# ethz-asl/okvis

Hardware: AMD Instinct MI355X
Metric: Gauss-Newton iterations/sec on 10-KF x 2-cam x 400-landmark windows (batch throughput: window-iterations/s) (higher is better)
Workload: dtype f64

## Files before the change

okvis_amd/csrc/ba_linearize2.hpp:

```cpp
#pragma once
#include "ba_linearize.hpp"

namespace ba {

constexpr int LIN2_REC = 27;
constexpr int LIN2_POSES = 64;
constexpr int LIN2_CAMS = 8;
constexpr int LIN2_IDX_INTS = 2 * (((GROUP_LM + 1) + 2 * LIN2_PIECES + LIN_TASK_CACHE * 6 + LIN2_PIECES / 2 + LIN2_PIECES / 4 + LIN2_CAMS + 1) / 2);

template <class REAL, bool FUSE, int UB = LIN2_REC>
struct Lin2Cfg {
  static constexpr int PAIR_REC_DOUBLES = (LIN2_PIECES * (UB > 16 ? UB : 16) * (int)sizeof(REAL) + 7) / 8;
  static constexpr int STAGE = LinCfg<false, REAL>::STAGE_DOUBLES;
  static constexpr int REC_DOUBLES = FUSE ? (STAGE > PAIR_REC_DOUBLES ? STAGE : PAIR_REC_DOUBLES) : PAIR_REC_DOUBLES;
  static constexpr int FIXED_DOUBLES = REC_DOUBLES + GROUP_LM * 4 + GROUP_LM * 16 + 4 * 64 + LIN2_POSES * 7 + LIN2_CAMS * 12 + LIN2_IDX_INTS / 2;
  static constexpr int MIN_STEP_DOUBLES = FUSE ? 1024 : 0;
};
static_assert(LIN2_PIECES * 3 * 2 <= LIN2_PIECES * 16, "phase A's pair sums alias the record area");
static_assert(LIN2_PIECES <= LIN_THREADS, "one pair per work-item");
__device__ __forceinline__ float fma_real(float a, float b, float c) { return fmaf(a, b, c); }
__device__ __forceinline__ double fma_real(double a, double b, double c) { return fma(a, b, c); }
template <class T>
__device__ __forceinline__ T sub_of_rounded_products(T a, T b, T c, T d) {
#pragma clang fp contract(off)
  const T p = a * b, q = c * d;
  return p - q;
}

template <class T>
__device__ __forceinline__ T row_next(T v) { return quad_xchg<0x101>(v); }
__device__ __forceinline__ int row_next_i(int v, int old) { return __builtin_amdgcn_update_dpp(old, v, 0x101, 0xF, 0xF, false); }
__device__ __forceinline__ int row_prev_i(int v, int old) { return __builtin_amdgcn_update_dpp(old, v, 0x111, 0xF, 0xF, false); }

struct Lin2Ops {
  ObsRec rec;
  int lpb, pp, poff, plm, pblock, slot;
  Task task;
};
struct Lin2Heavy {
  double Wp0[18];
  double bb[3], v[6], xx[4], sl[3];
  int lp0, lp1;
};

template <class REAL, bool FUSE, bool SMALL, int OCC = 2, int UB = LIN2_REC>
__global__ __launch_bounds__(LIN_THREADS, OCC) void linearize2_kernel(const WinPtrs* __restrict__ wins, const OptD* __restrict__ optp, int init,
                                                                      int n_small, int step_doubles) {
  extern __shared__ __attribute__((aligned(16))) double smem[];
  const WinPtrs& W = wins[blockIdx.y];
  int wg = blockIdx.x;
  if constexpr (SMALL) {
    if ((int)blockIdx.x < n_small) {
      small_body(W, init, blockIdx.x, smem);
      return;
    }
    wg -= n_small;
  }
  const int g = wg;
  if (g >= W.n_group) return;
#define LSTAMP(k) do { if (W.prof && threadIdx.x == 0 && g == 0) W.prof[k] = (double)clock64(); } while (0)
  const Ctrl* ctrl = W.ctrl;
  if (ctrl->done) return;
  const OptD opt = *optp;
  constexpr int RECD = Lin2Cfg<REAL, FUSE, UB>::REC_DOUBLES;
  REAL* s_rec = reinterpret_cast<REAL*>(smem);
  double* s_pair = smem;
  double* s_lm = smem + RECD;
  double* s_lmres = s_lm + GROUP_LM * 4;
  double* s_sc = s_lmres + GROUP_LM * 16;
  double* s_pose = s_sc + 4 * 64;
  double* s_cam = s_pose + LIN2_POSES * 7;
  int* s_lpb = reinterpret_cast<int*>(s_cam + LIN2_CAMS * 12);
  int* s_pp = s_lpb + GROUP_LM + 1;
  int* s_poff = s_pp + LIN2_PIECES;
  int* s_task = s_poff + LIN2_PIECES;
  int* s_cmodel = s_task + LIN_TASK_CACHE * 6;
  uint16_t* s_slot = reinterpret_cast<uint16_t*>(s_cmodel + LIN2_CAMS);
  uint8_t* s_plm = reinterpret_cast<uint8_t*>(s_slot + LIN2_PIECES);
  double* s_step = reinterpret_cast<double*>(s_lpb + LIN2_IDX_INTS);
  double* s_aux = s_step + (step_doubles - Lin2Cfg<REAL, FUSE, UB>::MIN_STEP_DOUBLES);
  const int tid = threadIdx.x, lane = tid & 63, wave = tid >> 6;

  auto reduce_own_group = [&](int g, int buf, double lam) {
    const Group Gr = W.groups[g];
    const int trows = min(TILE_DIM, W.Dp);
    double* tables = smem;
    double* aux = s_aux;
    double(*vinv)[6] = reinterpret_cast<double(*)[6]>(aux);
    double(*bvec)[3] = reinterpret_cast<double(*)[3]>(aux + SCHUR_CHUNK_LM_MAX * 6);
    int* boff = reinterpret_cast<int*>(aux + SCHUR_CHUNK_LM_MAX * 9);
    const SchurPairBeginGlobal pb{W.lm_pair_begin, Gr.lm_begin, Gr.lm_end};
    const int n_tp = W.n_tile * (W.n_tile + 1) / 2;
    for (int tp = 0; tp < n_tp; ++tp) {
      schur_reduce_chunk(W, opt, g, tp, Gr.lm_begin, Gr.lm_end, buf, lam, trows, tables, vinv, bvec, boff, pb, g == 0 && blockIdx.y == 0);
      __syncthreads();
    }
  };
  if (!init && !ctrl->pending) {
    if constexpr (FUSE)
      reduce_own_group(g, ctrl->acc, opt.dogleg ? ctrl->mu : 1.0 / ctrl->radius);
    return;
  }
  const int acc = ctrl->acc, trial = 1 - acc;
  const double lambda = ctrl->lambda;
  const double lam_next = opt.dogleg ? ((init || ctrl->first || opt.gauss_newton) ? ctrl->mu : fmax(DL_MIN_MU, 2.0 * ctrl->mu / DL_MU_INCREASE))
                                     : 1.0 / ctrl->radius;
  const bool dl_explicit = opt.dogleg && ctrl->tr_kind == 1;
  const double dl_cA = ctrl->cA, dl_beta = ctrl->beta;
  const bool fast = FUSE && W.fuse_fast;
  const bool poses_staged = W.n_pose <= LIN2_POSES, cams_staged = W.n_cam <= LIN2_CAMS;

  {
    const double* ps = W.pose[trial];
    const int np7 = 7 * min(W.n_pose, LIN2_POSES);
    for (int i = tid; i < np7; i += LIN_THREADS) s_pose[i] = ps[i];
    const int nc = min(W.n_cam, LIN2_CAMS);
    if (tid < 12 * nc) s_cam[tid] = W.cam_intr[tid];
    if (tid < nc) s_cmodel[tid] = W.cam_model[tid];
  }

  auto issue_loads = [&](const Group& G, Lin2Ops& o) {
    const int nlm = G.lm_end - G.lm_begin, nobs = G.obs_end - G.obs_begin, npair = G.pair_end - G.pair_begin, ntask = G.task_end - G.task_begin;
    o.rec.lm_cam = 0; o.rec.pose = 0; o.rec.ext = 0; o.rec.u = 0; o.rec.v = 0; o.rec.sw = 0;
    if (tid < nobs) o.rec = W.obs[G.obs_begin + tid];
    o.lpb = o.pp = o.poff = o.plm = o.pblock = o.slot = 0;
    if (tid <= nlm) o.lpb = W.lm_piece_begin[G.lm_begin + tid] - G.piece_begin;
    if (tid < npair) {
      o.pp = W.pair_piece[G.pair_begin + tid];
      o.poff = W.pair_off[G.pair_begin + tid];
      o.plm = W.pair_lm[G.pair_begin + tid] - G.lm_begin;
      o.pblock = W.pair_block[G.pair_begin + tid];
      o.slot = W.task_list[G.tlist_begin + tid];
    }
    if (ntask <= LIN_TASK_CACHE && tid < ntask) o.task = W.tasks[G.task_begin + tid];
  };
  auto issue_heavy = [&](const Group& G, Lin2Heavy& o) {
    const int nlm = G.lm_end - G.lm_begin, npair = G.pair_end - G.pair_begin;
    o.sl[0] = o.sl[1] = o.sl[2] = 1.0;
    o.lp0 = o.lp1 = 0;
    if (!init) {
      if (tid < npair) {
        const double* Wp = W.W[acc] + (size_t)(G.pair_begin + tid) * 18;
#pragma unroll
        for (int i = 0; i < 18; ++i) o.Wp0[i] = Wp[i];
      }
      if (tid < nlm) {
        const int l = G.lm_begin + tid;
        const double* b = W.bl[acc] + 3 * (size_t)l;
        const double* Vl = W.V[acc] + 6 * (size_t)l;
        const double* x = W.lm[acc] + 4 * (size_t)l;
#pragma unroll
        for (int i = 0; i < 3; ++i) o.bb[i] = b[i];
#pragma unroll
        for (int i = 0; i < 6; ++i) o.v[i] = Vl[i];
#pragma unroll
        for (int i = 0; i < 4; ++i) o.xx[i] = x[i];
        o.lp0 = W.lm_pair_begin[l] - G.pair_begin;
        o.lp1 = W.lm_pair_begin[l + 1] - G.pair_begin;
        if (opt.dogleg) {
          const double* sl = W.lm_scale + 3 * (size_t)l;
          o.sl[0] = sl[0], o.sl[1] = sl[1], o.sl[2] = sl[2];
        }
      }
    } else if (tid < nlm) {
      const double* x = W.lm[trial] + 4 * (size_t)(G.lm_begin + tid);
#pragma unroll
      for (int i = 0; i < 4; ++i) o.xx[i] = x[i];
    }
  };

  const Group G = W.groups[g];
  Lin2Ops ops;
  issue_loads(G, ops);
  if (!init)
    for (int i = tid; i < W.Dp; i += LIN_THREADS) s_step[i] = W.step[i];

  {
    LSTAMP(40);
    Lin2Heavy hv;
    issue_heavy(G, hv);
    const int nlm = G.lm_end - G.lm_begin;
    const int nobs = G.obs_end - G.obs_begin;
    const int npair = G.pair_end - G.pair_begin;
    const int ntask = G.task_end - G.task_begin;
    const bool has_obs = tid < nobs, has_pair = tid < npair;
    const bool tasks_cached = ntask <= LIN_TASK_CACHE;
    const ObsRec rec = ops.rec;
    const int pf_poff = ops.poff, pf_plm = ops.plm, pf_pblock = ops.pblock;
    double pf_sc[3] = {1.0, 1.0, 1.0};
    if (fast && !init && tid >= 64 && tid - 64 < nlm) {
      const double* sl = W.lm_scale + 3 * (size_t)(G.lm_begin + tid - 64);
      pf_sc[0] = sl[0], pf_sc[1] = sl[1], pf_sc[2] = sl[2];
    }
    LSTAMP(41);
    if (!init) {
      __syncthreads();
      if (has_pair) {
        const double* d = s_step + pf_poff;
        double t0 = 0, t1 = 0, t2 = 0;
#pragma unroll
        for (int i = 0; i < 6; ++i) {
          t0 += hv.Wp0[3 * i] * d[i];
          t1 += hv.Wp0[3 * i + 1] * d[i];
          t2 += hv.Wp0[3 * i + 2] * d[i];
        }
        s_pair[3 * tid] = t0;
        s_pair[3 * tid + 1] = t1;
        s_pair[3 * tid + 2] = t2;
      }
      __syncthreads();
      double sc_gd = 0, sc_ddd = 0, sc_s2 = 0, sc_x2 = 0;
      if (tid < nlm) {
        const int l = G.lm_begin + tid;
        double t[3] = {hv.bb[0], hv.bb[1], hv.bb[2]};
        for (int p = hv.lp0; p < hv.lp1; ++p) {
          const double* sp = s_pair + 3 * p;
          t[0] += sp[0];
          t[1] += sp[1];
          t[2] += sp[2];
        }
        double v[6] = {hv.v[0], hv.v[1], hv.v[2], hv.v[3], hv.v[4], hv.v[5]};
        const double d0 = damp_diag(v[0], hv.sl[0], opt);
        const double d1 = damp_diag(v[3], hv.sl[1], opt);
        const double d2 = damp_diag(v[5], hv.sl[2], opt);
        v[0] += lambda * d0;
        v[3] += lambda * d1;
        v[5] += lambda * d2;
        double vi[6];
        inv3sym(v, vi);
        const double dl0 = -(vi[0] * t[0] + vi[1] * t[1] + vi[2] * t[2]);
        const double dl1 = -(vi[1] * t[0] + vi[3] * t[1] + vi[4] * t[2]);
        const double dl2 = -(vi[2] * t[0] + vi[4] * t[1] + vi[5] * t[2]);
        double st0 = dl0, st1 = dl1, st2 = dl2;
        if (dl_explicit) {
          st0 = -dl_cA * (hv.bb[0] / d0) + dl_beta * dl0;
          st1 = -dl_cA * (hv.bb[1] / d1) + dl_beta * dl1;
          st2 = -dl_cA * (hv.bb[2] / d2) + dl_beta * dl2;
        }
        const double x0 = hv.xx[0], x1 = hv.xx[1], x2 = hv.xx[2], x3 = hv.xx[3];
        double* xt = W.lm[trial] + 4 * (size_t)l;
        const double n0 = x0 + st0, n1 = x1 + st1, n2 = x2 + st2;
        xt[0] = n0; xt[1] = n1; xt[2] = n2; xt[3] = x3;
        s_lm[4 * tid] = n0; s_lm[4 * tid + 1] = n1; s_lm[4 * tid + 2] = n2; s_lm[4 * tid + 3] = x3;
        sc_gd = hv.bb[0] * dl0 + hv.bb[1] * dl1 + hv.bb[2] * dl2;
        sc_ddd = d0 * dl0 * dl0 + d1 * dl1 * dl1 + d2 * dl2 * dl2;
        sc_s2 = st0 * st0 + st1 * st1 + st2 * st2;
        sc_x2 = x0 * x0 + x1 * x1 + x2 * x2 + x3 * x3;
      }
      if (tid < 64) {
        s_sc[tid] = sc_gd;
        s_sc[64 + tid] = sc_ddd;
        s_sc[128 + tid] = sc_s2;
        s_sc[192 + tid] = sc_x2;
      }
    } else {
      if (tid < nlm) {
        s_lm[4 * tid] = hv.xx[0]; s_lm[4 * tid + 1] = hv.xx[1]; s_lm[4 * tid + 2] = hv.xx[2]; s_lm[4 * tid + 3] = hv.xx[3];
      }
      if (tid < 64) s_sc[tid] = s_sc[64 + tid] = s_sc[128 + tid] = s_sc[192 + tid] = 0.0;
    }
    if (tid <= nlm) s_lpb[tid] = ops.lpb;
    if (has_pair) {
      s_pp[tid] = ops.pp;
      s_poff[tid] = pf_poff;
      s_plm[tid] = (uint8_t)pf_plm;
      s_slot[tid] = (uint16_t)ops.slot;
    }
    if (tasks_cached && tid < ntask) {
      int* t = s_task + 6 * tid;
      t[0] = ops.task.type; t[1] = ops.task.off_a; t[2] = ops.task.off_b;
      t[3] = ops.task.list_begin - G.tlist_begin; t[4] = ops.task.list_end - G.tlist_begin; t[5] = ops.task.out;
    }
    if (fast) {
      int* blktask = reinterpret_cast<int*>(s_aux + GROUP_LM * 9 + FUSE_MAX_TASKS * 36);
      if (tid >= 64 && tid < 64 + 32) blktask[tid - 64] = -1;
    }
    __syncthreads();
    LSTAMP(42);
    if (fast && tid < ntask) reinterpret_cast<int*>(s_aux + GROUP_LM * 9 + FUSE_MAX_TASKS * 36)[ops.task.off_a / 6] = tid;

    REAL a[16];
#pragma unroll
    for (int e = 0; e < 16; ++e) a[e] = REAL(0);
    const int key_l = has_obs ? (int)(rec.lm_cam & 0xFFFFFFu) : -1;
    const int key_p = has_obs ? (int)rec.pose : -1;
    if (has_obs) {
      const int o = G.obs_begin + tid;
      const int cam = (int)(rec.lm_cam >> 24);
      double P[7], E[7], intr[12];
      int cam_model;
      if (poses_staged) {
#pragma unroll
        for (int i = 0; i < 7; ++i) {
          P[i] = s_pose[7 * (int)rec.pose + i];
          E[i] = s_pose[7 * (int)rec.ext + i];
        }
      } else {
        const double* pose = W.pose[trial] + 7 * (size_t)rec.pose;
        const double* ext = W.pose[trial] + 7 * (size_t)rec.ext;
#pragma unroll
        for (int i = 0; i < 7; ++i) {
          P[i] = pose[i];
          E[i] = ext[i];
        }
      }
      if (cams_staged) {
#pragma unroll
        for (int i = 0; i < 12; ++i) intr[i] = s_cam[12 * cam + i];
        cam_model = s_cmodel[cam];
      } else {
#pragma unroll
        for (int i = 0; i < 12; ++i) intr[i] = W.cam_intr[12 * cam + i];
        cam_model = W.cam_model[cam];
      }
      const double* lm = s_lm + 4 * (key_l - G.lm_begin);
      const double L4[4] = {lm[0], lm[1], lm[2], lm[3]};
      REAL r0, r1, jl[6];
      if constexpr (std::is_same<REAL, double>::value) {
        ReprojLin Jd;
        reproj_linearize(P, E, L4, intr, cam_model, rec.u, rec.v, rec.sw, false, &Jd);
        r0 = Jd.r[0], r1 = Jd.r[1];
#pragma unroll
        for (int i = 0; i < 6; ++i) jl[i] = Jd.Jl[i];
      } else {
        ReprojLinT<REAL> J;
        reproj_linearize_mixed<REAL>(P, E, L4, intr, cam_model, rec.u, rec.v, rec.sw, false, &J);
        r0 = J.r[0], r1 = J.r[1];
#pragma unroll
        for (int i = 0; i < 6; ++i) jl[i] = J.Jl[i];
      }
      if (W.obs_r[trial]) {
        W.obs_r[trial][2 * (size_t)o] = r0;
        W.obs_r[trial][2 * (size_t)o + 1] = r1;
      }
      const REAL s = r0 * r0 + r1 * r1;
      REAL sr = REAL(1), irho = REAL(1), cost = REAL(0.5) * s;
      if (W.cauchy_b > 0) {
        const REAL bb = REAL(W.cauchy_b * W.cauchy_b);
        const REAL sum = REAL(1) + s / bb;
        const REAL rho1 = REAL(1) / sum;
        cost = REAL(0.5) * bb * log(sum);
        sr = sqrt(rho1);
        irho = sum;
      }
      r0 *= sr, r1 *= sr;
#pragma unroll
      for (int i = 0; i < 6; ++i) jl[i] *= sr;
      a[0] = jl[0] * jl[0] + jl[3] * jl[3];
      a[1] = jl[0] * jl[1] + jl[3] * jl[4];
      a[2] = jl[0] * jl[2] + jl[3] * jl[5];
      a[3] = jl[1] * jl[1] + jl[4] * jl[4];
      a[4] = jl[1] * jl[2] + jl[4] * jl[5];
      a[5] = jl[2] * jl[2] + jl[5] * jl[5];
      a[6] = jl[0] * r0 + jl[3] * r1;
      a[7] = jl[1] * r0 + jl[4] * r1;
      a[8] = jl[2] * r0 + jl[5] * r1;
#pragma unroll
      for (int e = 0; e < 6; ++e) a[9 + e] = a[e] * irho;
      a[15] = cost;
    }
    LSTAMP(43);
    const int prev_l = row_prev_i(key_l, -2), prev_p = row_prev_i(key_p, -2);
    const int next_l = row_next_i(key_l, -2), next_p = row_next_i(key_p, -2);
    const bool brk = ((lane & 15) == 0) | (key_l != prev_l) | (key_p != prev_p);
    const bool same_next = has_obs & ((lane & 15) != 15) & (key_l == next_l) & (key_p == next_p);
    const unsigned long long brk_mask = __ballot(brk);
    const unsigned long long below = brk_mask & ((2ull << lane) - 1ull);
    const int run_start = 63 - __builtin_clzll(below);
    const bool head = has_obs && (((lane - run_start) & 1) == 0);
    const bool merge = head && same_next;
    const unsigned long long head_mask = __ballot(head);
    const int pw = wave == 0 ? 0 : (wave == 1 ? G.pw1 : (wave == 2 ? G.pw2 : G.pw3));
    const int piece = pw + __builtin_amdgcn_mbcnt_hi((unsigned)(head_mask >> 32), __builtin_amdgcn_mbcnt_lo((unsigned)head_mask, 0));
#pragma unroll
    for (int e = 0; e < 16; ++e) {
      const REAL t = row_next(a[e]);
      a[e] += merge ? t : REAL(0);
    }
    if (head) {
      REAL* rp = s_rec + 16 * piece;
#pragma unroll
      for (int e = 0; e < 16; ++e) rp[e] = a[e];
    }
    __syncthreads();
    LSTAMP(44);

    {
      const int e = tid & 15;
      const bool is_cost = e == 15, is_b = e >= 6 && e < 9;
      double* obase = e < 6 ? W.V[trial] : (is_b ? W.bl[trial] : W.Hq[trial]);
      const int ostride = is_b ? 3 : 6, ooff = e < 6 ? e : (is_b ? e - 6 : e - 9);
      for (int wi = tid; wi < nlm * 16; wi += LIN_THREADS) {
        const int ll = wi >> 4;
        const int p0 = s_lpb[ll], p1 = s_lpb[ll + 1];
        REAL s0 = 0, s1 = 0;
        int p = p0;
        for (; p + 1 < p1; p += 2) {
          s0 += s_rec[16 * p + e];
          s1 += s_rec[16 * (p + 1) + e];
        }
        if (p < p1) s0 += s_rec[16 * p + e];
        const REAL sum = s0 + s1;
        if (!is_cost) obase[ostride * (size_t)(G.lm_begin + ll) + ooff] = sum;
        s_lmres[16 * ll + e] = sum;
        if (init && opt.dogleg && (e == 0 || e == 3 || e == 5))
          W.lm_scale[3 * (size_t)(G.lm_begin + ll) + (e == 0 ? 0 : (e == 3 ? 1 : 2))] = opt.jacobi_scaling ? 1.0 / (1.0 + sqrt((double)sum)) : 1.0;
      }
    }
    LSTAMP(45);
    REAL vp[6] = {0, 0, 0, 0, 0, 0}, bp[3] = {0, 0, 0};
    REAL d0 = 0, d1 = 0, d2 = 0, hw = 0;
    int my_slot = 0;
    if (has_pair) {
      const int pp = s_pp[tid];
      const int p0 = pp & 0xFFFF, p1 = p0 + (pp >> 16);
      for (int p = p0; p < p1; ++p) {
        const REAL* rp = s_rec + 16 * p;
#pragma unroll
        for (int e = 0; e < 6; ++e) vp[e] += rp[e];
#pragma unroll
        for (int e = 0; e < 3; ++e) bp[e] += rp[6 + e];
      }
      double pt[3];
      if (poses_staged) {
        pt[0] = s_pose[7 * pf_pblock], pt[1] = s_pose[7 * pf_pblock + 1], pt[2] = s_pose[7 * pf_pblock + 2];
      } else {
        const double* t = W.pose[trial] + 7 * (size_t)pf_pblock;
        pt[0] = t[0], pt[1] = t[1], pt[2] = t[2];
      }
      const double* x = s_lm + 4 * pf_plm;
      const double w = x[3];
      d0 = REAL(x[0] - pt[0] * w);
      d1 = REAL(x[1] - pt[1] * w);
      d2 = REAL(x[2] - pt[2] * w);
      hw = REAL(w);
      my_slot = (int)s_slot[tid];
    }
    __syncthreads();
    LSTAMP(46);
    if (wave == 3) {
      double cost = 0, gm = 0, sc_gd = 0, sc_ddd = 0, sc_s2 = 0, sc_x2 = 0;
      if (lane < nlm) {
        cost = s_lmres[16 * lane + 15];
        gm = fmax(fabs(s_lmres[16 * lane + 6]), fmax(fabs(s_lmres[16 * lane + 7]), fabs(s_lmres[16 * lane + 8])));
        sc_gd = s_sc[lane], sc_ddd = s_sc[64 + lane], sc_s2 = s_sc[128 + lane], sc_x2 = s_sc[192 + lane];
      }
      cost = wave_sum_full(cost);
      gm = wave_max_full(gm);
      sc_gd = wave_sum_full(sc_gd);
      sc_ddd = wave_sum_full(sc_ddd);
      sc_s2 = wave_sum_full(sc_s2);
      sc_x2 = wave_sum_full(sc_x2);
      if (lane == 0) {
        double* gs = W.gscal[trial] + (size_t)g * GS_COUNT;
        gs[GS_COST] = cost;
        gs[GS_GD] = sc_gd;
        gs[GS_DDD] = sc_ddd;
        gs[GS_STEP2] = sc_s2;
        gs[GS_X2] = sc_x2;
        gs[GS_GMAX] = gm;
      }
    }
    REAL Wm[18];
    {
      const REAL V3[3][3] = {{vp[0], vp[1], vp[2]}, {vp[1], vp[3], vp[4]}, {vp[2], vp[4], vp[5]}};
#pragma unroll
      for (int c = 0; c < 3; ++c) {
        Wm[0 + c] = -hw * V3[0][c];
        Wm[3 + c] = -hw * V3[1][c];
        Wm[6 + c] = -hw * V3[2][c];
        constexpr bool dbl = std::is_same<REAL, double>::value;
        if (dbl && c == 0) Wm[9 + c] = fma_real(-d1, V3[2][c], d2 * V3[1][c]);
        else Wm[9 + c] = fma_real(d2, V3[1][c], -(d1 * V3[2][c]));
        Wm[12 + c] = fma_real(d0, V3[2][c], -(d2 * V3[0][c]));
        if (dbl && c == 2) Wm[15 + c] = sub_of_rounded_products(d1, V3[0][c], d0, V3[1][c]);
        else Wm[15 + c] = fma_real(d1, V3[0][c], -(d0 * V3[1][c]));
      }
    }
    if (has_pair) {
      double* Wt = W.W[trial] + (size_t)(G.pair_begin + tid) * 18;
#pragma unroll
      for (int i = 0; i < 18; ++i) Wt[i] = Wm[i];
    }
    auto urec_k = [&](int kk) -> REAL {
      REAL v = 0;
      int k = 0;
#pragma unroll
      for (int ra = 0; ra < 7; ++ra)
#pragma unroll
        for (int b = (ra < 6 ? ra : 0); b < 6; ++b, ++k)
          if (k == kk) {
            const REAL w0 = ra < 6 ? Wm[3 * (ra < 6 ? ra : 0)] : bp[0], w1 = ra < 6 ? Wm[3 * (ra < 6 ? ra : 0) + 1] : bp[1],
                       w2 = ra < 6 ? Wm[3 * (ra < 6 ? ra : 0) + 2] : bp[2];
            if constexpr (std::is_same<REAL, float>::value)
              v = b == 0 ? -hw * w0 : b == 1 ? -hw * w1 : b == 2 ? -hw * w2 : b == 3 ? fmaf(w1, d2, -(w2 * d1)) : b == 4 ? fmaf(w2, d0, -(w0 * d2)) : fmaf(w0, d1, -(w1 * d0));
            else
              v = b == 0 ? -hw * w0 : b == 1 ? -hw * w1 : b == 2 ? -hw * w2 : b == 3 ? w1 * d2 - w2 * d1 : b == 4 ? w2 * d0 - w0 * d2 : w0 * d1 - w1 * d0;
          }
      return v;
    };
#pragma unroll
    for (int r0 = 0; r0 < LIN2_REC; r0 += UB) {
      const int ne = (LIN2_REC - r0 < UB) ? LIN2_REC - r0 : UB;
      if (r0 > 0) __syncthreads();
      if (has_pair) {
        REAL* ur = s_rec + UB * my_slot;
#pragma unroll
        for (int k = 0; k < UB; ++k)
          if (k < ne) ur[k] = urec_k(r0 + k);
      }
      __syncthreads();
      if (r0 == 0) LSTAMP(47);
      for (int wi = tid; wi < ntask * ne; wi += LIN_THREADS) {
        const int tt = wi / ne, k = wi - tt * ne;
        int lb, le, out;
        if (tasks_cached) {
          const int* t = s_task + 6 * tt;
          lb = t[3], le = t[4], out = t[5];
        } else {
          const Task T = W.tasks[G.task_begin + tt];
          lb = T.list_begin - G.tlist_begin, le = T.list_end - G.tlist_begin, out = T.out;
        }
        REAL s0 = 0, s1 = 0;
        int j = lb;
        for (; j + 1 < le; j += 2) {
          s0 += s_rec[j * UB + k];
          s1 += s_rec[(j + 1) * UB + k];
        }
        if (j < le) s0 += s_rec[j * UB + k];
        const REAL sum = s0 + s1;
        W.gpart[trial][out + r0 + k] = sum;
        if (fast) s_aux[GROUP_LM * 9 + tt * 36 + r0 + k] = sum;
      }
    }
    LSTAMP(48);
    LSTAMP(49);
    if constexpr (FUSE) {
      __syncthreads();
      if (fast) {
        FuseItemsT<6> fit;
#pragma unroll
        for (int q = 0; q < 6; ++q) {
          fit.row[q] = has_pair ? pf_poff + q : -1;
          fit.lm[q] = pf_plm;
          fit.w[q][0] = Wm[3 * q], fit.w[q][1] = Wm[3 * q + 1], fit.w[q][2] = Wm[3 * q + 2];
        }
        fused_reduce_fast<RECD, 6>(W, opt, g, trial, lam_next, nlm, init != 0, pf_sc, fit, smem, s_lmres, s_aux);
      } else {
        reduce_own_group(g, trial, lam_next);
      }
    }
    LSTAMP(50);
    LSTAMP(51);
  }
#undef LSTAMP
}

__global__ __launch_bounds__(LIN_THREADS, 2) void small_kernel(const WinPtrs* __restrict__ wins, int init) {
  extern __shared__ __attribute__((aligned(16))) double smem[];
  small_body(wins[blockIdx.y], init, blockIdx.x, smem);
}
__global__ __launch_bounds__(LIN_THREADS, 2) void small_prepare_kernel(const WinPtrs* __restrict__ wins) {
  extern __shared__ __attribute__((aligned(16))) double smem[];
  small_body<1>(wins[blockIdx.y], 0, blockIdx.x, smem);
}

__global__ __launch_bounds__(IMU_THREADS, 2) void imu_pre_kernel(const WinPtrs* __restrict__ mini, const double* __restrict__ sb0s) {
  extern __shared__ __attribute__((aligned(16))) double smem[];
  imu_redo(mini[blockIdx.x], 0, sb0s + 9 * (size_t)blockIdx.x, smem, threadIdx.x);
}
__global__ void imu_pre_place_kernel(const WinPtrs* __restrict__ wins, const int2* __restrict__ where, const ImuCacheD* __restrict__ src) {
  const int2 wf = where[blockIdx.x];
  const double* s = reinterpret_cast<const double*>(src + blockIdx.x);
  auto d = reinterpret_cast<BA_G double*>(wins[wf.x].imu_cache + wf.y);
  for (int i = threadIdx.x; i < (int)(sizeof(ImuCacheD) / 8) - 1; i += blockDim.x) d[i] = s[i];
  if (threadIdx.x == 0) {
    wins[wf.x].imu_cache[wf.y].valid = 3;
    wins[wf.x].imu_cache[wf.y].redo_count = 1;
  }
}

}
```

okvis_amd/csrc/capi_launch.inc:

```
namespace {

size_t lin_smem(bool ext, bool f32 = false) {
  const int d = f32 ? (ext ? LinCfg<true, float>::SMEM_DOUBLES : LinCfg<false, float>::SMEM_DOUBLES)
                    : (ext ? LinCfg<true, double>::SMEM_DOUBLES : LinCfg<false, double>::SMEM_DOUBLES);
  return (size_t)d * sizeof(double);
}
size_t solve_smem(int Dpad, bool large) {
  return ((large ? 0 : (size_t)ldl16_area_doubles(Dpad)) + 4 * (size_t)Dpad) * sizeof(double) + 16;
}
size_t solve_smem_chain(int chain_doubles, int Dpad) { return ((size_t)chain_doubles + 4 * (size_t)Dpad) * sizeof(double) + 16; }
int lin2_step_doubles(int max_Dp, bool fuse, bool f32) {
  const int aux = fuse ? (f32 ? Lin2Cfg<float, true>::MIN_STEP_DOUBLES : Lin2Cfg<double, true>::MIN_STEP_DOUBLES) : Lin2Cfg<double, false>::MIN_STEP_DOUBLES;
  return ((max_Dp + 1) / 2) * 2 + 8 + aux;
}
size_t lin2_smem(int max_Dp, bool fuse, bool f32, bool two_rounds = false) {
  const int fixed = two_rounds ? (f32 ? Lin2Cfg<float, false, 14>::FIXED_DOUBLES : Lin2Cfg<double, false, 14>::FIXED_DOUBLES)
                    : f32 ? (fuse ? Lin2Cfg<float, true>::FIXED_DOUBLES : Lin2Cfg<float, false>::FIXED_DOUBLES)
                          : (fuse ? Lin2Cfg<double, true>::FIXED_DOUBLES : Lin2Cfg<double, false>::FIXED_DOUBLES);
  return (size_t)(fixed + lin2_step_doubles(max_Dp, fuse, f32)) * sizeof(double);
}
size_t small_smem() { return (size_t)std::max<int>(std::max<int>(ImuLds::TOTAL, EvalLds::TOTAL), 2 * MAX_MARG_DIM) * sizeof(double); }

size_t small_eval_smem() { return (size_t)std::max<int>(EvalLds::TOTAL, 2 * MAX_MARG_DIM) * sizeof(double); }

int sch2_serial_nlb(int trows) {
  const int nlb = sch2_nlb(trows, 5120);
  return nlb < 12 ? sch2_nlb(trows, 9216) : nlb;
}

std::vector<std::pair<const void*, size_t>> plan_kernels() {
  auto f = [](auto k) { return reinterpret_cast<const void*>(k); };
  const size_t dense = std::max(solve_smem(((MAX_D_LDS + 5) / 6) * 6, false), (size_t)SOLVE_LDS_LIMIT), chain = SOLVE_LDS_LIMIT_CHAIN;
  size_t wide = 0;
  for (int t = 1; t <= TILE_DIM; ++t) wide = std::max(wide, (size_t)sch2_tile_doubles(t, sch2_serial_nlb(t)) * sizeof(double));
  const size_t d = std::max(lin2_smem(MAX_D, true, false), small_smem()), s = std::max(lin2_smem(MAX_D, true, true), small_smem());
  const size_t ef = std::max(lin_smem(true, true), small_smem()), ed = std::max(lin_smem(true), small_smem());
  const size_t pf = std::max(lin_smem(false, true), small_smem()), pd = std::max(lin_smem(false), small_smem());
  return {{f(&solve_kernel<false, true, true>), chain}, {f(&solve_kernel<false, false, true>), chain},
          {f(&solve_kernel<false, true>), dense}, {f(&solve_kernel<false, false>), dense},
          {f(&schur_ride_kernel<3>), std::max(wide, small_eval_smem())}, {f(&schur_mfma_kernel<3>), wide}, {f(&schur_mfma_kernel<9>), wide},
          {f(&schur_kernel), 2 * SCHUR_LM_BATCH * TILE_DIM * 3 * sizeof(double)},
          {f(&solve_kernel<true, false>), solve_smem(((MAX_D + 5) / 6) * 6, true)},
          {f(&small_kernel), small_smem()}, {f(&small_prepare_kernel), small_smem()},
          {f(&linearize2_kernel<float, true, false>), s}, {f(&linearize2_kernel<float, false, false, 4, 14>), s},
          {f(&linearize2_kernel<float, false, false, 3>), s}, {f(&linearize2_kernel<double, true, false>), d},
          {f(&linearize2_kernel<double, false, false, 4, 14>), d}, {f(&linearize2_kernel<double, false, false, 3>), d},
          {f(&linearize2_kernel<float, true, true>), s}, {f(&linearize2_kernel<float, false, true>), s},
          {f(&linearize2_kernel<double, true, true>), d}, {f(&linearize2_kernel<double, false, true>), d},
          {f(&linearize_kernel<true, float, true>), ef}, {f(&linearize_kernel<true, float, false>), ef},
          {f(&linearize_kernel<true, double, true>), ed}, {f(&linearize_kernel<true, double, false>), ed},
          {f(&linearize_kernel<false, float, true>), pf}, {f(&linearize_kernel<false, float, false>), pf},
          {f(&linearize_kernel<false, double, true>), pd}, {f(&linearize_kernel<false, double, false>), pd},
          {f(&schur_ride_kernel<3, true>), std::max(wide, small_eval_smem())}, {f(&schur_mfma_kernel<3, true>), wide}};
}

using LinFn = decltype(&linearize_kernel<false, double, false>);
using Lin2Fn = decltype(&linearize2_kernel<double, false, true>);
using SolveFn = decltype(&solve_kernel<false, false>);
const LinFn LIN[8] = {&linearize_kernel<false, double, false>, &linearize_kernel<false, double, true>, &linearize_kernel<false, float, false>,
                      &linearize_kernel<false, float, true>,   &linearize_kernel<true, double, false>,  &linearize_kernel<true, double, true>,
                      &linearize_kernel<true, float, false>,   &linearize_kernel<true, float, true>};
enum { LIN2_FUSED, LIN2_FUSED_SMALL, LIN2_SMALL, LIN2_OCC3, LIN2_OCC4 };
const Lin2Fn LIN2[10] = {&linearize2_kernel<double, true, false>, &linearize2_kernel<double, true, true>, &linearize2_kernel<double, false, true>,
                         &linearize2_kernel<double, false, false, 3>, &linearize2_kernel<double, false, false, 4, 14>,
                         &linearize2_kernel<float, true, false>, &linearize2_kernel<float, true, true>, &linearize2_kernel<float, false, true>,
                         &linearize2_kernel<float, false, false, 3>, &linearize2_kernel<float, false, false, 4, 14>};
enum { SOLVE_NONE, SOLVE_DENSE, SOLVE_DENSE_DBUF, SOLVE_CHAIN, SOLVE_CHAIN_DBUF, SOLVE_TILED };
const SolveFn SOLVE[6] = {nullptr, &solve_kernel<false, false>, &solve_kernel<false, true>, &solve_kernel<false, false, true>,
                          &solve_kernel<false, true, true>, &solve_kernel<true, false>};
enum { SCHUR_NONE, SCHUR_VALU, SCHUR_MFMA3, SCHUR_MFMA9, SCHUR_RIDE3, SCHUR_MFMA3_SERIAL, SCHUR_RIDE3_SERIAL };
enum { SMALL_NONE, SMALL_ALL, SMALL_PREPARE };
LaunchPlan make_plan(const BatchLayout& L, const BatchMax& M, const okvis_ba_options& o, int n_windows) {
  LaunchPlan p;
  const bool f32 = o.fp32_linearize != 0;
  p.fused = M.group_chunks && f32 == L.fp32 && decision_free(o);
  p.nodec = M.spec_schur && !p.fused && decision_free(o);
  p.lin2 = L.lin2, p.split_small = L.split_small, p.graph = o.use_graph != 0;
  p.n_small = M.imu + 1;
  p.trows = std::min(TILE_DIM, M.Dp);
  if (M.schur_blocks > 0 && !p.fused) {
    const bool small_tiles = schur_small_tiles(M.Dp);
    if (!M.any_ext && schur_mfma_allowed(o) && (small_tiles || (o.tuning.flags & OKVIS_BA_TUNE_SCHUR_MFMA_LARGE))) {
      p.nlb = sch2_serial_nlb(p.trows);
      const bool serial = !small_tiles || (o.tuning.flags & OKVIS_BA_TUNE_SCHUR_SERIAL_BATCHES);
      if (!serial) p.nlb = SCH2_STAGE_LM;
      const int sm = (serial ? sch2_tile_doubles(p.trows, p.nlb) : sch2_ring_doubles(p.trows)) * (int)sizeof(double);
      p.rides = small_tiles && p.nodec && L.split_small && !(o.tuning.flags & OKVIS_BA_TUNE_NO_SMALL_RIDE);
      if (p.rides) p.schur = Launch{serial ? SCHUR_RIDE3_SERIAL : SCHUR_RIDE3, p.n_small + M.schur_blocks, std::max(sm, (int)small_eval_smem())};
      else p.schur = Launch{!small_tiles ? SCHUR_MFMA9 : serial ? SCHUR_MFMA3_SERIAL : SCHUR_MFMA3, M.schur_blocks, sm};
    } else {
      p.schur = Launch{SCHUR_VALU, M.schur_blocks, (int)(2 * SCHUR_LM_BATCH * p.trows * 3 * sizeof(double))};
    }
  }
  if (M.Dpad_small > 0)
    p.solve = Launch{(M.chain ? SOLVE_CHAIN : SOLVE_DENSE) + (M.group_chunks || M.spec_schur), 0,
                     (int)(M.chain ? solve_smem_chain(M.chain_doubles, M.Dpad_small) : solve_smem(M.Dpad_small, false))};
  if (M.Dpad_large > 0) {
    p.tiled = Launch{SOLVE_TILED, 0, (int)solve_smem(M.Dpad_large, true)};
    p.nT = (M.Dpad_large + CT_TB - 1) / CT_TB;
  }
  const Launch small{SMALL_ALL, p.n_small, (int)small_smem()};
  if (L.lin2) {
    const int t = f32 ? 5 : 0, smem2 = (int)lin2_smem(M.Dp, p.fused, f32);
    p.sd = lin2_step_doubles(M.Dp, p.fused, f32);
    if (L.split_small) {
      p.small_init = small;
      p.small_iter = !p.rides ? small : M.imu > 0 ? Launch{SMALL_PREPARE, M.imu, (int)small_smem()} : Launch{};
      const int occ = o.tuning.lin2_occupancy > 0 ? o.tuning.lin2_occupancy : 4;
      const bool two_rounds = !p.fused && occ >= 4;
      p.lin = Launch{t + (p.fused ? LIN2_FUSED : occ >= 4 ? LIN2_OCC4 : LIN2_OCC3), M.group,
                     two_rounds ? (int)lin2_smem(M.Dp, false, f32, true) : smem2};
    } else {
      p.lin = Launch{t + (p.fused ? LIN2_FUSED_SMALL : LIN2_SMALL), p.n_small + M.group, std::max(smem2, (int)small_smem())};
      p.lin_n_small = p.n_small;
    }
  } else {
    p.lin = Launch{4 * M.any_ext + 2 * f32 + p.fused, p.n_small + M.group, (int)std::max(lin_smem(M.any_ext, f32), small_smem())};
    p.lin_n_small = p.n_small;
  }
  if (M.imu > 0 && o.strategy == OKVIS_BA_STRATEGY_DOGLEG && !o.gauss_newton) p.take_back = Launch{1, M.imu, 0};
  p.budget = o.strategy == OKVIS_BA_STRATEGY_DOGLEG;
  int nsub = o.n_streams > 0 ? o.n_streams : (n_windows >= 128 ? 2 : (n_windows >= 56 ? 3 : (n_windows >= 8 ? 2 : 1)));
  nsub = std::max(1, std::min(nsub, n_windows));
  auto extent = [](int w0, int nw) { return Extent{w0, nw, nw <= SOLVE_HELPED_MAX_WINDOWS ? SOLVE_HELPERS : 0}; };
  for (int k = 0; k < nsub; ++k) {
    const int w0 = (int)((int64_t)n_windows * k / nsub), w1 = (int)((int64_t)n_windows * (k + 1) / nsub);
    p.subs.push_back(extent(w0, w1 - w0));
  }
  p.whole = extent(0, n_windows);
  p.one_helpers = extent(0, 1).helpers;
  return p;
}

__global__ void begin_kernel(const WinPtrs* wins, const int* accs, double initial_radius) {
  const WinPtrs& W = wins[blockIdx.x];
  const int acc = accs[blockIdx.x], tr = 1 - acc, tid = threadIdx.x;
  for (int i = tid; i < 7 * W.n_pose; i += blockDim.x) W.pose[tr][i] = W.pose[acc][i];
  for (int i = tid; i < 9 * W.n_sb; i += blockDim.x) W.sb[tr][i] = W.sb[acc][i];
  for (int i = tid; i < 4 * W.n_lm; i += blockDim.x) W.lm[tr][i] = W.lm[acc][i];
  if (tid == 0) {
    Ctrl c;
    for (size_t k = 0; k < sizeof(Ctrl) / 8; ++k) reinterpret_cast<double*>(&c)[k] = 0.0;
    c.acc = acc;
    c.pending = 1;
    c.first = 1;
    c.radius = initial_radius;
    c.decrease_factor = 2.0;
    c.lambda = 1.0 / initial_radius;
    c.mu = DL_MIN_MU;
    *W.ctrl = c;
  }
}
__global__ void gather_ctrl_kernel(const WinPtrs* wins, Ctrl* out, int n) {
  const int w = blockIdx.x * (blockDim.x / 64) + threadIdx.x / 64, lane = threadIdx.x & 63;
  if (w < n && lane < (int)(sizeof(Ctrl) / 8))
    reinterpret_cast<double*>(out + w)[lane] = reinterpret_cast<const double*>(wins[w].ctrl)[lane];
}

__global__ void delay_kernel(long long ticks) {
  const long long t0 = wall_clock64();
  while (wall_clock64() - t0 < ticks) __builtin_amdgcn_s_sleep(32);
}

struct Sub { hipStream_t st; int w0, nw, helpers; };
Sub sub(hipStream_t st, const Extent& e) { return Sub{st, e.w0, e.nw, e.helpers}; }
Sub whole(okvis_ba_solver* s) { return sub(s->stream, s->plan.whole); }

hipError_t launch_schur(okvis_ba_solver* s, Sub b, int final_call = 0) {
  const LaunchPlan& p = s->plan;
  const dim3 grid((unsigned)p.schur.gx, (unsigned)b.nw), blk(SCHUR_THREADS);
  const WinPtrs* wins = s->d_wins + b.w0;
  const CtrlSlot* ctrls = s->d_ctrl + b.w0;
  switch (p.schur.k) {
    case SCHUR_NONE: return hipSuccess;
    case SCHUR_VALU: hipLaunchKernelGGL(schur_kernel, grid, blk, p.schur.lds, b.st, wins, s->d_opt, p.trows, final_call); break;
    case SCHUR_MFMA3: hipLaunchKernelGGL(schur_mfma_kernel<3>, grid, blk, p.schur.lds, b.st, wins, s->d_opt, p.trows, final_call, p.nlb, ctrls, p.nodec); break;
    case SCHUR_MFMA9: hipLaunchKernelGGL(schur_mfma_kernel<9>, grid, blk, p.schur.lds, b.st, wins, s->d_opt, p.trows, final_call, p.nlb, ctrls, p.nodec); break;
    case SCHUR_RIDE3: hipLaunchKernelGGL(schur_ride_kernel<3>, grid, blk, p.schur.lds, b.st, wins, s->d_opt, p.trows, final_call, p.nlb, ctrls, p.nodec, p.n_small); break;
    case SCHUR_MFMA3_SERIAL: hipLaunchKernelGGL((schur_mfma_kernel<3, true>), grid, blk, p.schur.lds, b.st, wins, s->d_opt, p.trows, final_call, p.nlb, ctrls, p.nodec); break;
    case SCHUR_RIDE3_SERIAL: hipLaunchKernelGGL((schur_ride_kernel<3, true>), grid, blk, p.schur.lds, b.st, wins, s->d_opt, p.trows, final_call, p.nlb, ctrls, p.nodec, p.n_small); break;
  }
  return hipGetLastError();
}
void launch_solve_kernel(okvis_ba_solver* s, const Launch& l, dim3 grid, hipStream_t st, const WinPtrs* wins, int final_only, CtrlSlot* ctrls) {
  const SolveFn fn = SOLVE[l.k];
  hipLaunchKernelGGL(fn, grid, dim3(SOLVE_THREADS), l.lds, st, wins, s->d_opt, final_only, ctrls);
}
hipError_t launch_solve(okvis_ba_solver* s, Sub b, int final_only) {
  const LaunchPlan& p = s->plan;
  if (p.solve.k) launch_solve_kernel(s, p.solve, dim3((unsigned)b.nw, 1 + b.helpers), b.st, s->d_wins + b.w0, final_only, s->d_ctrl + b.w0);
  if (p.tiled.k) {
    launch_solve_kernel(s, p.tiled, dim3((unsigned)b.nw), b.st, s->d_wins + b.w0, final_only, s->d_ctrl + b.w0);
    if (!final_only) {
      const int nT = p.nT;
      hipLaunchKernelGGL(large_export_kernel, dim3(nT * (nT + 1) / 2, (unsigned)b.nw, CT_TILE / CT_THREADS), dim3(CT_THREADS), 0, b.st,
                         s->d_wins + b.w0);
      hipLaunchKernelGGL(chol_tiles_window_kernel, dim3(nT * (nT + 1) / 2 + nT, (unsigned)b.nw), dim3(CT_THREADS), CT_SMEM_DOUBLES * 8,
                         b.st, s->d_wins + b.w0);
      hipLaunchKernelGGL(solve_large_tail_kernel, dim3((unsigned)b.nw), dim3(SOLVE_THREADS), 0, b.st, s->d_wins + b.w0, s->d_opt);
    }
  }
  return hipGetLastError();
}
hipError_t launch_lin(okvis_ba_solver* s, Sub b, int init) {
  const LaunchPlan& p = s->plan;
  const WinPtrs* wins = s->d_wins + b.w0;
  const Launch& f = init ? p.small_init : p.small_iter;
  if (f.k == SMALL_ALL) hipLaunchKernelGGL(small_kernel, dim3((unsigned)f.gx, (unsigned)b.nw), dim3(LIN_THREADS), f.lds, b.st, wins, init);
  if (f.k == SMALL_PREPARE) hipLaunchKernelGGL(small_prepare_kernel, dim3((unsigned)f.gx, (unsigned)b.nw), dim3(LIN_THREADS), f.lds, b.st, wins);
  const dim3 grid((unsigned)p.lin.gx, (unsigned)b.nw);
  if (p.lin2) {
    const Lin2Fn fn = LIN2[p.lin.k];
    hipLaunchKernelGGL(fn, grid, dim3(LIN_THREADS), p.lin.lds, b.st, wins, s->d_opt, init, p.lin_n_small, p.sd);
  } else {
    const LinFn fn = LIN[p.lin.k];
    hipLaunchKernelGGL(fn, grid, dim3(LIN_THREADS), p.lin.lds, b.st, wins, s->d_opt, init, p.lin_n_small);
  }
  return hipGetLastError();
}
hipError_t launch_imu_take_back(okvis_ba_solver* s, int w0, int nw) {
  if (!s->plan.take_back.k) return hipSuccess;
  hipLaunchKernelGGL(imu_take_back_kernel, dim3((unsigned)s->plan.take_back.gx, (unsigned)nw), dim3(64), 0, s->stream, s->d_wins + w0);
  return hipGetLastError();
}
hipError_t launch_iteration(okvis_ba_solver* s, Sub b) {
  hipError_t e;
  if ((e = launch_schur(s, b)) != hipSuccess) return e;
  if ((e = launch_solve(s, b, 0)) != hipSuccess) return e;
  return launch_lin(s, b, 0);
}
hipError_t launch_budget(okvis_ba_solver* s, Sub b, int n) {
  if (!s->plan.budget || n <= 0) return hipSuccess;
  hipLaunchKernelGGL(add_budget_kernel, dim3((unsigned)b.nw), dim3(64), 0, b.st, s->d_wins + b.w0, n);
  return hipGetLastError();
}
hipError_t launch_chain(okvis_ba_solver* s, Sub b, int n, int budget) {
  hipError_t e = launch_budget(s, b, budget);
  for (int i = 0; i < n && e == hipSuccess; ++i) e = launch_iteration(s, b);
  return e;
}
hipError_t launch_iterations_forked(okvis_ba_solver* s, int n, int budget = -1) {
  const int nsub = (int)s->sub_streams.size();
  if (budget < 0) budget = n;
  if (nsub <= 1) return launch_chain(s, whole(s), n, budget);
  hipError_t e = hipEventRecord(s->ev_fork, s->stream);
  for (int k = 0; k < nsub && e == hipSuccess; ++k) {
    e = hipStreamWaitEvent(s->sub_streams[k], s->ev_fork, 0);
    if (e == hipSuccess) e = launch_chain(s, sub(s->sub_streams[k], s->plan.subs[k]), n, budget);
    if (e == hipSuccess) e = hipEventRecord(s->sub_events[k], s->sub_streams[k]);
    if (e == hipSuccess) e = hipStreamWaitEvent(s->stream, s->sub_events[k], 0);
  }
  return e;
}

int refresh_acc(okvis_ba_solver* s, int w) {
  if (s->acc_fresh) return OKVIS_BA_OK;
  int acc = 0;
  HIP_TRY(hipMemcpyAsync(&acc, &s->wins[w].ptrs.ctrl->acc, sizeof(int), hipMemcpyDeviceToHost, s->stream));
  HIP_TRY(hipStreamSynchronize(s->stream));
  s->wins[w].acc = acc & 1;
  return OKVIS_BA_OK;
}

hipError_t reserve_ctrl_stage(okvis_ba_solver* s, size_t n_windows) {
  const size_t bytes = std::max(sizeof(Ctrl), sizeof(int)) * n_windows;
  if (bytes <= s->ctrl_stage_bytes) return hipSuccess;
  if (s->h_ctrl_stage) (void)hipHostFree(s->h_ctrl_stage);
  if (s->d_ctrl_stage) (void)hipFree(s->d_ctrl_stage);
  s->h_ctrl_stage = s->d_ctrl_stage = nullptr;
  s->ctrl_stage_bytes = 0;
  hipError_t e = hipHostMalloc((void**)&s->h_ctrl_stage, bytes, hipHostMallocDefault);
  if (e == hipSuccess) e = hipMalloc((void**)&s->d_ctrl_stage, bytes);
  if (e == hipSuccess) s->ctrl_stage_bytes = bytes;
  return e;
}

int fetch_ctrl(okvis_ba_solver* s, std::vector<Ctrl>& out) {
  const size_t n = s->wins.size();
  out.resize(n);
  HIP_TRY(reserve_ctrl_stage(s, n));
  hipLaunchKernelGGL(gather_ctrl_kernel, dim3((unsigned)((n + 3) / 4)), dim3(256), 0, s->stream, s->d_wins, reinterpret_cast<Ctrl*>(s->d_ctrl_stage), (int)n);
  HIP_TRY(hipGetLastError());
  HIP_TRY(hipMemcpyAsync(s->h_ctrl_stage, s->d_ctrl_stage, sizeof(Ctrl) * n, hipMemcpyDeviceToHost, s->stream));
  HIP_TRY(hipStreamSynchronize(s->stream));
  std::memcpy(out.data(), s->h_ctrl_stage, sizeof(Ctrl) * n);
  return OKVIS_BA_OK;
}

}
```

Before: 541,800.

## Hoist and batch all linearize2 global loads ahead of first use

The linearize2 kernel now issues every per-block global load up front, before any dependent work. That covers control state, a touch of each cache line of WinPtrs/OptD, the staged poses, intrinsics, step vector, obs records, pair metadata, and the heavy W/V/b/x data. Masked lanes are redirected to a safe dummy address rather than branched around, so the loads can be issued unconditionally and overlap in flight. Control is read from a per-window slot passed as a new kernel argument instead of through W.ctrl, and the profiling timestamps are captured in registers. The aim is to cut serialized load latency at kernel start, at the cost of more registers and possible occupancy pressure.

New measurement: 535,700. 1.1% lower.

```diff
diff --git a/okvis_amd/csrc/ba_linearize2.hpp b/okvis_amd/csrc/ba_linearize2.hpp
--- a/okvis_amd/csrc/ba_linearize2.hpp
+++ b/okvis_amd/csrc/ba_linearize2.hpp
@@ -45,8 +45,9 @@
 
 template <class REAL, bool FUSE, bool SMALL, int OCC = 2, int UB = LIN2_REC>
 __global__ __launch_bounds__(LIN_THREADS, OCC) void linearize2_kernel(const WinPtrs* __restrict__ wins, const OptD* __restrict__ optp, int init,
-                                                                      int n_small, int step_doubles) {
+                                                                      int n_small, int step_doubles, const CtrlSlot* __restrict__ ctrls) {
   extern __shared__ __attribute__((aligned(16))) double smem[];
+  const long long t_start = clock64();
   const WinPtrs& W = wins[blockIdx.y];
   int wg = blockIdx.x;
   if constexpr (SMALL) {
@@ -57,11 +58,33 @@
     wg -= n_small;
   }
   const int g = wg;
+  const Ctrl* ctrl = &ctrls[blockIdx.y].c;
+  typedef int lin2_i4 __attribute__((ext_vector_type(4)));
+  const lin2_i4 chead = *reinterpret_cast<const lin2_i4*>(ctrl);
+  const double c_lambda = ctrl->lambda, c_mu = ctrl->mu, c_radius = ctrl->radius, c_cA = ctrl->cA, c_beta = ctrl->beta;
+  const int c_tr_kind = ctrl->tr_kind;
+  const OptD& opt = *optp;
+  constexpr int lines = (int)((sizeof(WinPtrs) + 63) / 64), olines = (int)((sizeof(OptD) + 63) / 64);
+  static_assert(sizeof(WinPtrs) % 4 == 0 && (lines - 1) * 64 < (int)sizeof(WinPtrs) && (olines - 1) * 64 < (int)sizeof(OptD), "lines touched below");
+  int wv[lines], ov[olines];
+  {
+    const int* wi = reinterpret_cast<const int*>(&W);
+    const int* oi = reinterpret_cast<const int*>(optp);
+#pragma unroll
+    for (int k = 0; k < lines; ++k) wv[k] = wi[16 * k];
+#pragma unroll
+    for (int k = 0; k < olines; ++k) ov[k] = oi[16 * k];
+  }
+  __builtin_amdgcn_sched_barrier(0);
+  int warm = chead.w | c_tr_kind | __double2loint(c_lambda) | __double2loint(c_mu) | __double2loint(c_radius) | __double2loint(c_cA) | __double2loint(c_beta);
+#pragma unroll
+  for (int k = 0; k < lines; ++k) warm |= wv[k];
+#pragma unroll
+  for (int k = 0; k < olines; ++k) warm |= ov[k];
+  if ((init == 0x7ffffff1) & (warm == 0x5a5a5a5a)) return;
   if (g >= W.n_group) return;
 #define LSTAMP(k) do { if (W.prof && threadIdx.x == 0 && g == 0) W.prof[k] = (double)clock64(); } while (0)
-  const Ctrl* ctrl = W.ctrl;
-  if (ctrl->done) return;
-  const OptD opt = *optp;
+  if (chead.w) return;
   constexpr int RECD = Lin2Cfg<REAL, FUSE, UB>::REC_DOUBLES;
   REAL* s_rec = reinterpret_cast<REAL*>(smem);
   double* s_pair = smem;
@@ -96,103 +119,99 @@
       __syncthreads();
     }
   };
-  if (!init && !ctrl->pending) {
+  if (!init && !chead.y) {
     if constexpr (FUSE)
-      reduce_own_group(g, ctrl->acc, opt.dogleg ? ctrl->mu : 1.0 / ctrl->radius);
+      reduce_own_group(g, chead.x, opt.dogleg ? c_mu : 1.0 / c_radius);
     return;
   }
-  const int acc = ctrl->acc, trial = 1 - acc;
-  const double lambda = ctrl->lambda;
-  const double lam_next = opt.dogleg ? ((init || ctrl->first || opt.gauss_newton) ? ctrl->mu : fmax(DL_MIN_MU, 2.0 * ctrl->mu / DL_MU_INCREASE))
-                                     : 1.0 / ctrl->radius;
-  const bool dl_explicit = opt.dogleg && ctrl->tr_kind == 1;
-  const double dl_cA = ctrl->cA, dl_beta = ctrl->beta;
+  const int acc = chead.x, trial = 1 - acc;
+  const double lambda = c_lambda;
+  const double lam_next = opt.dogleg ? ((init || chead.z || opt.gauss_newton) ? c_mu : fmax(DL_MIN_MU, 2.0 * c_mu / DL_MU_INCREASE))
+                                     : 1.0 / c_radius;
+  const bool dl_explicit = opt.dogleg && c_tr_kind == 1;
+  const double dl_cA = c_cA, dl_beta = c_beta;
   const bool fast = FUSE && W.fuse_fast;
   const bool poses_staged = W.n_pose <= LIN2_POSES, cams_staged = W.n_cam <= LIN2_CAMS;
 
+  const Group G = W.groups[g];
+  static_assert(sizeof(WinPtrs) >= sizeof(double) * 18 && sizeof(WinPtrs) >= sizeof(ObsRec) && sizeof(WinPtrs) >= sizeof(Task), "the largest request `there` redirects");
+  auto there = [&](auto p, bool on) { return on ? p : (decltype(p))as_global(&W); };
+  static_assert(7 * LIN2_POSES <= 2 * LIN_THREADS && 12 * LIN2_CAMS <= LIN_THREADS, "the staged poses take two values per work-item, the intrinsics one");
+  const int np7 = 7 * min(W.n_pose, LIN2_POSES), nc = min(W.n_cam, LIN2_CAMS), Dp = W.Dp;
+  const bool step_staged = !init && Dp > 0;
+  auto g_pose = there(W.pose[trial], np7 > 0);
+  auto g_step = there(W.step, step_staged);
+  const double st_pose0 = g_pose[tid < np7 ? tid : 0], st_pose1 = g_pose[tid + LIN_THREADS < np7 ? tid + LIN_THREADS : 0];
+  const double st_intr = there(W.cam_intr, nc > 0)[tid < 12 * nc ? tid : 0];
+  const int st_model = there(W.cam_model, nc > 0)[tid < nc ? tid : 0];
+  const double st_step0 = g_step[(step_staged && tid < Dp) ? tid : 0], st_step1 = g_step[(step_staged && tid + LIN_THREADS < Dp) ? tid + LIN_THREADS : 0];
+
+  const int nlm = G.lm_end - G.lm_begin;
+  const int nobs = G.obs_end - G.obs_begin;
+  const int npair = G.pair_end - G.pair_begin;
+  const int ntask = G.task_end - G.task_begin;
+  const bool has_obs = tid < nobs, has_pair = tid < npair, has_lm = tid < nlm;
+  const bool tasks_cached = ntask <= LIN_TASK_CACHE;
+  const size_t l_req = has_lm ? (size_t)(G.lm_begin + tid) : (size_t)0;
+  const size_t p_req = has_pair ? (size_t)(G.pair_begin + tid) : (size_t)0;
+  Lin2Ops ops;
+  ops.rec = there(W.obs, nobs > 0)[has_obs ? G.obs_begin + tid : 0];
+  ops.lpb = W.lm_piece_begin[tid <= nlm ? G.lm_begin + tid : 0];
+  ops.pp = there(W.pair_piece, npair > 0)[p_req];
+  ops.poff = there(W.pair_off, npair > 0)[p_req];
+  ops.plm = there(W.pair_lm, npair > 0)[p_req];
+  ops.pblock = there(W.pair_block, npair > 0)[p_req];
+  ops.slot = there(W.task_list, npair > 0)[has_pair ? G.tlist_begin + tid : 0];
+  ops.task = there(W.tasks, tasks_cached && ntask > 0)[tasks_cached && tid < ntask ? G.task_begin + tid : 0];
+  const long long t_40 = clock64();
+  Lin2Heavy hv;
+  hv.lp0 = hv.lp1 = 0;
+  if (!init) {
+    auto Wp = there(W.W[acc], npair > 0) + p_req * 18;
+#pragma unroll
+    for (int i = 0; i < 18; ++i) hv.Wp0[i] = Wp[i];
+    auto b = W.bl[acc] + 3 * l_req;
+    auto Vl = W.V[acc] + 6 * l_req;
+    auto x = W.lm[acc] + 4 * l_req;
+#pragma unroll
+    for (int i = 0; i < 3; ++i) hv.bb[i] = b[i];
+#pragma unroll
+    for (int i = 0; i < 6; ++i) hv.v[i] = Vl[i];
+#pragma unroll
+    for (int i = 0; i < 4; ++i) hv.xx[i] = x[i];
+    hv.lp0 = W.lm_pair_begin[l_req];
+    hv.lp1 = W.lm_pair_begin[l_req + 1];
+  } else {
+    auto x = W.lm[trial] + 4 * l_req;
+#pragma unroll
+    for (int i = 0; i < 4; ++i) hv.xx[i] = x[i];
+  }
+  const bool sl_there = !init && opt.dogleg;
   {
-    const double* ps = W.pose[trial];
-    const int np7 = 7 * min(W.n_pose, LIN2_POSES);
-    for (int i = tid; i < np7; i += LIN_THREADS) s_pose[i] = ps[i];
-    const int nc = min(W.n_cam, LIN2_CAMS);
-    if (tid < 12 * nc) s_cam[tid] = W.cam_intr[tid];
-    if (tid < nc) s_cmodel[tid] = W.cam_model[tid];
-  }
-
-  auto issue_loads = [&](const Group& G, Lin2Ops& o) {
-    const int nlm = G.lm_end - G.lm_begin, nobs = G.obs_end - G.obs_begin, npair = G.pair_end - G.pair_begin, ntask = G.task_end - G.task_begin;
-    o.rec.lm_cam = 0; o.rec.pose = 0; o.rec.ext = 0; o.rec.u = 0; o.rec.v = 0; o.rec.sw = 0;
-    if (tid < nobs) o.rec = W.obs[G.obs_begin + tid];
-    o.lpb = o.pp = o.poff = o.plm = o.pblock = o.slot = 0;
-    if (tid <= nlm) o.lpb = W.lm_piece_begin[G.lm_begin + tid] - G.piece_begin;
-    if (tid < npair) {
-      o.pp = W.pair_piece[G.pair_begin + tid];
-      o.poff = W.pair_off[G.pair_begin + tid];
-      o.plm = W.pair_lm[G.pair_begin + tid] - G.lm_begin;
-      o.pblock = W.pair_block[G.pair_begin + tid];
-      o.slot = W.task_list[G.tlist_begin + tid];
-    }
-    if (ntask <= LIN_TASK_CACHE && tid < ntask) o.task = W.tasks[G.task_begin + tid];
-  };
-  auto issue_heavy = [&](const Group& G, Lin2Heavy& o) {
-    const int nlm = G.lm_end - G.lm_begin, npair = G.pair_end - G.pair_begin;
-    o.sl[0] = o.sl[1] = o.sl[2] = 1.0;
-    o.lp0 = o.lp1 = 0;
-    if (!init) {
-      if (tid < npair) {
-        const double* Wp = W.W[acc] + (size_t)(G.pair_begin + tid) * 18;
-#pragma unroll
-        for (int i = 0; i < 18; ++i) o.Wp0[i] = Wp[i];
-      }
-      if (tid < nlm) {
-        const int l = G.lm_begin + tid;
-        const double* b = W.bl[acc] + 3 * (size_t)l;
-        const double* Vl = W.V[acc] + 6 * (size_t)l;
-        const double* x = W.lm[acc] + 4 * (size_t)l;
-#pragma unroll
-        for (int i = 0; i < 3; ++i) o.bb[i] = b[i];
-#pragma unroll
-        for (int i = 0; i < 6; ++i) o.v[i] = Vl[i];
-#pragma unroll
-        for (int i = 0; i < 4; ++i) o.xx[i] = x[i];
-        o.lp0 = W.lm_pair_begin[l] - G.pair_begin;
-        o.lp1 = W.lm_pair_begin[l + 1] - G.pair_begin;
-        if (opt.dogleg) {
-          const double* sl = W.lm_scale + 3 * (size_t)l;
-          o.sl[0] = sl[0], o.sl[1] = sl[1], o.sl[2] = sl[2];
-        }
-      }
-    } else if (tid < nlm) {
-      const double* x = W.lm[trial] + 4 * (size_t)(G.lm_begin + tid);
-#pragma unroll
-      for (int i = 0; i < 4; ++i) o.xx[i] = x[i];
-    }
-  };
-
-  const Group G = W.groups[g];
-  Lin2Ops ops;
-  issue_loads(G, ops);
-  if (!init)
-    for (int i = tid; i < W.Dp; i += LIN_THREADS) s_step[i] = W.step[i];
+    auto sl = there(W.lm_scale, sl_there) + 3 * (sl_there ? l_req : (size_t)0);
+    hv.sl[0] = sl[0], hv.sl[1] = sl[1], hv.sl[2] = sl[2];
+  }
+  double pf_sc[3];
+  const bool sc_lane = tid >= 64 && tid - 64 < nlm;
+  if constexpr (FUSE) {
+    const bool sc_there = fast && !init;
+    auto sl = there(W.lm_scale, sc_there) + 3 * (size_t)(sc_there && sc_lane ? G.lm_begin + tid - 64 : 0);
+    pf_sc[0] = sl[0], pf_sc[1] = sl[1], pf_sc[2] = sl[2];
+  }
+  const long long t_41 = clock64();
 
   {
-    LSTAMP(40);
-    Lin2Heavy hv;
-    issue_heavy(G, hv);
-    const int nlm = G.lm_end - G.lm_begin;
-    const int nobs = G.obs_end - G.obs_begin;
-    const int npair = G.pair_end - G.pair_begin;
-    const int ntask = G.task_end - G.task_begin;
-    const bool has_obs = tid < nobs, has_pair = tid < npair;
-    const bool tasks_cached = ntask <= LIN_TASK_CACHE;
     const ObsRec rec = ops.rec;
-    const int pf_poff = ops.poff, pf_plm = ops.plm, pf_pblock = ops.pblock;
-    double pf_sc[3] = {1.0, 1.0, 1.0};
-    if (fast && !init && tid >= 64 && tid - 64 < nlm) {
-      const double* sl = W.lm_scale + 3 * (size_t)(G.lm_begin + tid - 64);
-      pf_sc[0] = sl[0], pf_sc[1] = sl[1], pf_sc[2] = sl[2];
-    }
-    LSTAMP(41);
+    const int pf_poff = has_pair ? ops.poff : 0, pf_plm = has_pair ? ops.plm - G.lm_begin : 0, pf_pblock = has_pair ? ops.pblock : 0;
+    if (tid < np7) s_pose[tid] = st_pose0;
+    if (tid + LIN_THREADS < np7) s_pose[tid + LIN_THREADS] = st_pose1;
+    if (tid < 12 * nc) s_cam[tid] = st_intr;
+    if (tid < nc) s_cmodel[tid] = st_model;
+    if (step_staged) {
+      if (tid < Dp) s_step[tid] = st_step0;
+      if (tid + LIN_THREADS < Dp) s_step[tid + LIN_THREADS] = st_step1;
+      for (int i = tid + 2 * LIN_THREADS; i < Dp; i += LIN_THREADS) s_step[i] = W.step[i];
+    }
     if (!init) {
       __syncthreads();
       if (has_pair) {
@@ -213,7 +232,7 @@
       if (tid < nlm) {
         const int l = G.lm_begin + tid;
         double t[3] = {hv.bb[0], hv.bb[1], hv.bb[2]};
-        for (int p = hv.lp0; p < hv.lp1; ++p) {
+        for (int p = hv.lp0 - G.pair_begin; p < hv.lp1 - G.pair_begin; ++p) {
           const double* sp = s_pair + 3 * p;
           t[0] += sp[0];
           t[1] += sp[1];
@@ -259,7 +278,7 @@
       }
       if (tid < 64) s_sc[tid] = s_sc[64 + tid] = s_sc[128 + tid] = s_sc[192 + tid] = 0.0;
     }
-    if (tid <= nlm) s_lpb[tid] = ops.lpb;
+    if (tid <= nlm) s_lpb[tid] = ops.lpb - G.piece_begin;
     if (has_pair) {
       s_pp[tid] = ops.pp;
       s_poff[tid] = pf_poff;
@@ -276,6 +295,11 @@
       if (tid >= 64 && tid < 64 + 32) blktask[tid - 64] = -1;
     }
     __syncthreads();
+    if (W.prof && tid == 0 && g == 0) {
+      W.prof[52] = (double)t_start;
+      W.prof[40] = (double)t_40;
+      W.prof[41] = (double)t_41;
+    }
     LSTAMP(42);
     if (fast && tid < ntask) reinterpret_cast<int*>(s_aux + GROUP_LM * 9 + FUSE_MAX_TASKS * 36)[ops.task.off_a / 6] = tid;
 
@@ -545,6 +569,7 @@
           fit.lm[q] = pf_plm;
           fit.w[q][0] = Wm[3 * q], fit.w[q][1] = Wm[3 * q + 1], fit.w[q][2] = Wm[3 * q + 2];
         }
+        if (!(sc_lane && !init)) pf_sc[0] = pf_sc[1] = pf_sc[2] = 1.0;
         fused_reduce_fast<RECD, 6>(W, opt, g, trial, lam_next, nlm, init != 0, pf_sc, fit, smem, s_lmres, s_aux);
       } else {
         reduce_own_group(g, trial, lam_next);
diff --git a/okvis_amd/csrc/capi_launch.inc b/okvis_amd/csrc/capi_launch.inc
--- a/okvis_amd/csrc/capi_launch.inc
+++ b/okvis_amd/csrc/capi_launch.inc
@@ -211,7 +211,8 @@
   const dim3 grid((unsigned)p.lin.gx, (unsigned)b.nw);
   if (p.lin2) {
     const Lin2Fn fn = LIN2[p.lin.k];
-    hipLaunchKernelGGL(fn, grid, dim3(LIN_THREADS), p.lin.lds, b.st, wins, s->d_opt, init, p.lin_n_small, p.sd);
+    const CtrlSlot* ctrls = s->d_ctrl + b.w0;
+    hipLaunchKernelGGL(fn, grid, dim3(LIN_THREADS), p.lin.lds, b.st, wins, s->d_opt, init, p.lin_n_small, p.sd, ctrls);
   } else {
     const LinFn fn = LIN[p.lin.k];
     hipLaunchKernelGGL(fn, grid, dim3(LIN_THREADS), p.lin.lds, b.st, wins, s->d_opt, init, p.lin_n_small);
```
